# zju3dv/LoG

Measured on NVIDIA H100. Metric: gaussians_per_s_fwd_bwd, higher is better.
Workload: dtype f32

## Files before the change

### log_b200/csrc/lgr_blend.cu

```cuda
#include "lgr_common.cuh"
#include "lgr_prof.cuh"

namespace lgr {

constexpr int BLEND_THREADS = TILE_PIX;
#ifndef LGR_FWD_MIN_CTAS
#define LGR_FWD_MIN_CTAS 5
#endif
#ifndef LGR_BWD_MIN_CTAS
#define LGR_BWD_MIN_CTAS 4
#endif
#ifndef LGR_FWD6_MIN_CTAS
#define LGR_FWD6_MIN_CTAS 4
#endif
#ifndef LGR_BWD6_MIN_CTAS
#define LGR_BWD6_MIN_CTAS 3
#endif
constexpr int BATCH = 256;
constexpr unsigned FULL = 0xffffffffu;

struct SubTile {
  int x, y;
  bool inside;
};

__device__ __forceinline__ SubTile make_subtile(const View& v, int tile, int lane, int warp) {
  SubTile s;
  const int tx = tile % v.gx, ty = v.row0 + tile / v.gx;
  const int sx = tx * TILE + (warp & 1) * 8, sy = ty * TILE + (warp >> 1) * 4;
  s.x = sx + (lane & 7); s.y = sy + (lane >> 3);
  s.inside = s.x < v.W && s.y < v.H;
  return s;
}

__device__ __forceinline__ unsigned subtile_bits(const float4 r0, const float4 r1, float tx0, float ty0) {
  const float xlo = r0.x - r1.z, xhi = r0.x + r1.z, ylo = r0.y - r1.w, yhi = r0.y + r1.w;
  unsigned xm = 0u, m = 0u;
  if (xhi >= tx0 && xlo <= tx0 + 7.0f) xm |= 1u;
  if (xhi >= tx0 + 8.0f && xlo <= tx0 + 15.0f) xm |= 2u;
#pragma unroll
  for (int r = 0; r < 4; r++)
    if (yhi >= ty0 + 4.0f * r && ylo <= ty0 + 4.0f * r + 3.0f) m |= xm << (2 * r);
  return m;
}

__device__ __forceinline__ float eval_power2(const float4 r0, const float con_z, float dx, float dy) {
  const float q = __fmaf_rn(r0.z, __fmul_rn(dx, dx), __fmul_rn(con_z, __fmul_rn(dy, dy)));
  return __fmaf_rn(-0.5f, q, -__fmul_rn(r0.w, __fmul_rn(dx, dy)));
}
__device__ __forceinline__ float ex2_approx(float x) {
  float y;
  asm("ex2.approx.ftz.f32 %0, %1;" : "=f"(y) : "f"(x));
  return y;
}
__device__ __forceinline__ float eval_alpha(float opacity, float G) { return fminf(ALPHA_MAX, __fmul_rn(opacity, G)); }

__device__ __forceinline__ uint32_t smem_u32(const void* p) { return (uint32_t)__cvta_generic_to_shared(p); }
__device__ __forceinline__ float4 lds_f4(uint32_t addr) {
  float4 v;
  asm volatile("ld.shared.v4.f32 {%0, %1, %2, %3}, [%4];" : "=f"(v.x), "=f"(v.y), "=f"(v.z), "=f"(v.w) : "r"(addr));
  return v;
}
__device__ __forceinline__ float2 lds_f2(uint32_t addr) {
  float2 v;
  asm volatile("ld.shared.v2.f32 {%0, %1}, [%2];" : "=f"(v.x), "=f"(v.y) : "r"(addr));
  return v;
}
__device__ __forceinline__ uint32_t pin_reg(uint32_t v) {
  asm volatile("" : "+r"(v));
  return v;
}
__device__ __forceinline__ void red_shared_max_u32(uint32_t addr, unsigned v) {
  asm volatile("red.shared.max.u32 [%0], %1;" ::"r"(addr), "r"(v) : "memory");
}
__device__ __forceinline__ void red_shared_add_f32(uint32_t addr, float v) {
  asm volatile("red.shared.add.f32 [%0], %1;" ::"r"(addr), "f"(v) : "memory");
}
__device__ __forceinline__ void sts_f32(uint32_t addr, float v) {
  asm volatile("st.shared.f32 [%0], %1;" ::"r"(addr), "f"(v) : "memory");
}
__device__ __forceinline__ float rcp_approx(float x) {
  float y;
  asm("rcp.approx.ftz.f32 %0, %1;" : "=f"(y) : "f"(x));
  return y;
}
__device__ __forceinline__ void prefetch_l2(const float* p) {
  asm volatile("prefetch.global.L2 [%0];" ::"l"(p));
}
__device__ __forceinline__ float tf32_lo(float x) { return x - __uint_as_float(__float_as_uint(x) & 0xffffe000u); }
__device__ __forceinline__ void ldsm_x4(uint32_t addr, uint32_t& r0, uint32_t& r1, uint32_t& r2, uint32_t& r3) {
  asm volatile("ldmatrix.sync.aligned.m8n8.x4.shared.b16 {%0, %1, %2, %3}, [%4];"
               : "=r"(r0), "=r"(r1), "=r"(r2), "=r"(r3) : "r"(addr));
}
__device__ __forceinline__ void mma_tf32(float& d0, float& d1, float& d2, float& d3, uint32_t a0, uint32_t a1, uint32_t a2,
                                         uint32_t a3, uint32_t b0, uint32_t b1) {
  asm volatile("mma.sync.aligned.m16n8k8.row.col.f32.tf32.tf32.f32 {%0, %1, %2, %3}, {%4, %5, %6, %7}, {%8, %9}, {%0, %1, %2, %3};"
               : "+f"(d0), "+f"(d1), "+f"(d2), "+f"(d3) : "r"(a0), "r"(a1), "r"(a2), "r"(a3), "r"(b0), "r"(b1));
}

template <bool SIX = false>
__device__ __forceinline__ void stage_splat(float4* s_rec, unsigned char* s_bits, int slot, const float* __restrict__ splat,
                                            int id, float tx0, float ty0, const uint32_t* __restrict__ recorded = nullptr,
                                            const float* __restrict__ splat_ext = nullptr) {
  constexpr int F4 = SIX ? 4 : 3;
  const float* rec = splat + (int64_t)id * LGR_SPLAT_FLOATS;
  const float4 r0 = ldg4(rec);
  float4 r1 = ldg4(rec + 4), r2 = ldg4(rec + 8);
  float4 r3;
  if (SIX) r3 = ldg4(splat_ext + 4 * (int64_t)id);
  r2.w = __int_as_float(id);
  unsigned bits;
  if (recorded) {
    const uint32_t e = *recorded;
    bits = e & 0xffu;
    r1.z = __uint_as_float(e >> 8);
  } else {
    bits = subtile_bits(r0, r1, tx0, ty0);
  }
  s_rec[F4 * slot] = r0; s_rec[F4 * slot + 1] = r1; s_rec[F4 * slot + 2] = r2;
  if (SIX) s_rec[F4 * slot + 3] = r3;
  s_bits[slot] = (unsigned char)bits;
}

template <bool AUX, bool REC, bool SIX = false>
__global__ void __launch_bounds__(BLEND_THREADS, SIX ? LGR_FWD6_MIN_CTAS : LGR_FWD_MIN_CTAS)
blend_fwd_kernel(View v, const int32_t* __restrict__ tile_start, const int32_t* __restrict__ sorted_ids,
                 const float* __restrict__ splat, float* __restrict__ image, float* __restrict__ final_T,
                 int32_t* __restrict__ n_contrib, int32_t* __restrict__ pid_pixel, float* __restrict__ pw_pixel,
                 unsigned* __restrict__ point_weight_bits, int32_t* __restrict__ point_count) {
  constexpr int F4 = SIX ? 4 : 3;
  constexpr uint32_t RB = 16u * F4;
  __shared__ float4 s_rec[BATCH * F4];
  __shared__ unsigned s_w[AUX ? BATCH : 1];
  __shared__ unsigned char s_bits[BATCH];
  __shared__ unsigned s_cb[REC ? (BLEND_THREADS / 32) * (BATCH / 32) : 1];
  const int tile = blockIdx.x, tid = threadIdx.x, lane = tid & 31, warp = tid >> 5;
  const SubTile st = make_subtile(v, tile, lane, warp);
  const float pxf = (float)st.x, pyf = (float)st.y;
  const float tx0 = (float)((tile % v.gx) * TILE), ty0 = (float)((v.row0 + tile / v.gx) * TILE);
  const int beg = tile_start[tile], len = tile_start[tile + 1] - beg;
  const uint32_t s_w_addr = smem_u32(s_w);
  const uint32_t s_rec_addr = pin_reg(smem_u32(s_rec));

  float T = 1.0f, C0 = 0.f, C1 = 0.f, C2 = 0.f, wmax = 0.f;
  float C3 = 0.f, C4 = 0.f, C5 = 0.f;
  int last = 0, wid = -1;
  int done = st.inside ? 0 : 1;
  int id_next = tid < len ? sorted_ids[beg + tid] : -1;

  int base = 0, cnt = min(BATCH, len);
  int n_rec = 0;
  auto stage = [&]() {
    if (tid < cnt) stage_splat<SIX>(s_rec, s_bits, tid, splat, id_next, tx0, ty0, nullptr, v.splat_ext);
    else s_bits[tid] = 0;
    if (AUX) s_w[tid] = 0u;
    id_next = base + BATCH + tid < len ? sorted_ids[beg + base + BATCH + tid] : -1;
    if (id_next >= 0) prefetch_l2(splat + (int64_t)id_next * LGR_SPLAT_FLOATS);
    if (SIX && id_next >= 0) prefetch_l2(v.splat_ext + 4 * (int64_t)id_next);
  };
  if (len > 0) stage();
  while (base < len) {
    __syncthreads();
    if (REC) {
      if (lane < BATCH / 32) s_cb[warp * (BATCH / 32) + lane] = 0u;
      __syncwarp();
    }
    if (!__all_sync(FULL, done)) {
      for (int c0 = 0; c0 < cnt; c0 += 32) {
        const int e_l = c0 + lane;
        unsigned mask = __ballot_sync(FULL, (s_bits[e_l] >> warp) & 1u);
        unsigned own_w = 0u;
        unsigned took = 0u;
        while (mask) {
          const int jA = __ffs(mask) - 1;
          mask &= mask - 1;
          const bool two = mask != 0u;
          const int jB = two ? __ffs(mask) - 1 : jA;
          mask &= mask - 1;
          const uint32_t recA = s_rec_addr + RB * (uint32_t)(c0 + jA), recB = s_rec_addr + RB * (uint32_t)(c0 + jB);
          const float4 r0A = lds_f4(recA), r0B = lds_f4(recB);
          const float2 r1A = lds_f2(recA + 16u), r1B = lds_f2(recB + 16u);
          const float dxA = __fsub_rn(r0A.x, pxf), dyA = __fsub_rn(r0A.y, pyf);
          const float dxB = __fsub_rn(r0B.x, pxf), dyB = __fsub_rn(r0B.y, pyf);
          const float powerA = eval_power2(r0A, r1A.x, dxA, dyA), powerB = eval_power2(r0B, r1B.x, dxB, dyB);
          const float alphaA = eval_alpha(r1A.y, ex2_approx(powerA)), alphaB = eval_alpha(r1B.y, ex2_approx(powerB));
          float wA = 0.f, wB = 0.f;
          if (!done && powerA <= 0.0f && alphaA >= ALPHA_MIN) {
            const float test_T = __fmul_rn(T, __fsub_rn(1.0f, alphaA));
            if (test_T < T_STOP) done = 1;
            else {
              wA = alphaA * T;
              const float4 r2 = lds_f4(recA + 32u);
              C0 = fmaf(r2.x, wA, C0); C1 = fmaf(r2.y, wA, C1); C2 = fmaf(r2.z, wA, C2);
              if (SIX) {
                const float4 r3 = lds_f4(recA + 48u);
                C3 = fmaf(r3.x, wA, C3); C4 = fmaf(r3.y, wA, C4); C5 = fmaf(r3.z, wA, C5);
              }
              T = test_T;
              last = base + c0 + jA + 1;
              if (AUX && wA > wmax) { wmax = wA; wid = __float_as_int(r2.w); }
            }
          }
          if (two && !done && powerB <= 0.0f && alphaB >= ALPHA_MIN) {
            const float test_T = __fmul_rn(T, __fsub_rn(1.0f, alphaB));
            if (test_T < T_STOP) done = 1;
            else {
              wB = alphaB * T;
              const float4 r2 = lds_f4(recB + 32u);
              C0 = fmaf(r2.x, wB, C0); C1 = fmaf(r2.y, wB, C1); C2 = fmaf(r2.z, wB, C2);
              if (SIX) {
                const float4 r3 = lds_f4(recB + 48u);
                C3 = fmaf(r3.x, wB, C3); C4 = fmaf(r3.y, wB, C4); C5 = fmaf(r3.z, wB, C5);
              }
              T = test_T;
              last = base + c0 + jB + 1;
              if (AUX && wB > wmax) { wmax = wB; wid = __float_as_int(r2.w); }
            }
          }
          if (AUX) {
            const unsigned mA = __reduce_max_sync(FULL, __float_as_uint(wA));
            const unsigned mB = __reduce_max_sync(FULL, __float_as_uint(wB));
            if (lane == jA) own_w = mA;
            if (two && lane == jB) own_w = mB;
          } else if (REC) {
            if (__any_sync(FULL, wA != 0.f)) took |= 1u << jA;
            if (__any_sync(FULL, wB != 0.f)) took |= 1u << jB;
          }
        }
        if (AUX && REC) took = __ballot_sync(FULL, own_w != 0u);
        if (REC && lane == 0) s_cb[warp * (BATCH / 32) + (c0 >> 5)] = took;
        if (AUX && own_w) red_shared_max_u32(s_w_addr + 4u * e_l, own_w);
        if (__all_sync(FULL, done)) break;
      }
    }
    const int all_done = __syncthreads_and(done);
    if (AUX && tid < cnt && s_w[tid]) atomicMax(point_weight_bits + __float_as_int(s_rec[F4 * tid + 2].w), s_w[tid]);
    if (REC) {
      unsigned m = 0u;
      if (lane < BATCH / 32) {
#pragma unroll
        for (int w = 0; w < BLEND_THREADS / 32; w++) m |= s_cb[w * (BATCH / 32) + lane];
      }
      const int c = __popc(m);
      int incl = c;
#pragma unroll
      for (int d = 1; d < BATCH / 32; d <<= 1) {
        const int y = __shfl_up_sync(FULL, incl, d);
        if (lane >= d) incl += y;
      }
      const unsigned mine = __shfl_sync(FULL, m, warp);
      const int before = __shfl_sync(FULL, incl - c, warp);
      if ((mine >> lane) & 1u) {
        unsigned byte = 0u;
#pragma unroll
        for (int w = 0; w < BLEND_THREADS / 32; w++) byte |= ((s_cb[w * (BATCH / 32) + warp] >> lane) & 1u) << w;
        const int k = beg + n_rec + before + __popc(mine & ((1u << lane) - 1u));
        v.contrib_id[k] = __float_as_int(s_rec[F4 * tid + 2].w);
        v.contrib_entry[k] = byte | ((uint32_t)(base + tid) << 8);
      }
      n_rec += __shfl_sync(FULL, incl, BATCH / 32 - 1);
    }
    base += BATCH;
    if (all_done || base >= len) break;
    cnt = min(BATCH, len - base);
    stage();
  }
  if (REC && tid == 0) v.contrib_count[tile] = n_rec;
  if (st.inside) {
    const int64_t pix = (int64_t)st.y * v.W + st.x, HW = (int64_t)v.H * v.W;
    image[pix] = C0 + T * __ldg(v.bg);
    image[HW + pix] = C1 + T * __ldg(v.bg + 1);
    image[2 * HW + pix] = C2 + T * __ldg(v.bg + 2);
    if (SIX) {
      image[3 * HW + pix] = C3 + T * __ldg(v.bg + 3);
      image[4 * HW + pix] = C4 + T * __ldg(v.bg + 4);
      image[5 * HW + pix] = C5 + T * __ldg(v.bg + 5);
    }
    final_T[pix] = T;
    n_contrib[pix] = last;
    if (AUX) {
      pid_pixel[pix] = (v.pid_map && wid >= 0) ? v.pid_map[wid] : wid; pw_pixel[pix] = wmax;
      if (point_count && wid >= 0) atomicAdd(point_count + wid, 1);
    }
  }
}

constexpr int HITS = 8;
constexpr int XROW = 36;
constexpr int BWD_SMEM = BATCH * 48 + BATCH * 36 + (BLEND_THREADS / 32) * (2 * HITS * XROW + 192 + 192) * 4 + BATCH;
constexpr int BWD6_SMEM = BATCH * 64 + BATCH * 48 + (BLEND_THREADS / 32) * (2 * HITS * XROW + 384 + 192) * 4 + BATCH;

template <bool REC, bool SIX = false>
__global__ void __launch_bounds__(BLEND_THREADS, SIX ? LGR_BWD6_MIN_CTAS : LGR_BWD_MIN_CTAS)
blend_bwd_kernel(View v, const int32_t* __restrict__ tile_start, const int32_t* __restrict__ sorted_ids,
                 const float* __restrict__ splat, const float* __restrict__ image,
                 const float* __restrict__ dL_dimage, float* __restrict__ dsplat) {
  constexpr int F4 = SIX ? 4 : 3;
  constexpr uint32_t RB = 16u * F4;
  constexpr int NCH = SIX ? 6 : 3;
  constexpr int NG = 6 + NCH;
  constexpr int NCW = 64 * NCH;
  extern __shared__ float4 smem_f4[];
  float4* s_rec = smem_f4;
  float* s_g = reinterpret_cast<float*>(s_rec + BATCH * F4);
  float* s_x = s_g + BATCH * NG;
  float* s_cw = s_x + (BLEND_THREADS / 32) * 2 * HITS * XROW;
  float* s_mw = s_cw + (BLEND_THREADS / 32) * NCW;
  unsigned char* s_bits = reinterpret_cast<unsigned char*>(s_mw + (BLEND_THREADS / 32) * 192);
  const int tile = blockIdx.x, tid = threadIdx.x, lane = tid & 31, warp = tid >> 5;
  const SubTile st = make_subtile(v, tile, lane, warp);
  const float pxf = (float)st.x, pyf = (float)st.y;
  const float tx0 = (float)((tile % v.gx) * TILE), ty0 = (float)((v.row0 + tile / v.gx) * TILE);
  const int beg = tile_start[tile], len = tile_start[tile + 1] - beg;
  const uint32_t s_g_addr = pin_reg(smem_u32(s_g));
  const uint32_t s_rec_addr = pin_reg(smem_u32(s_rec));
  const uint32_t xg_addr = pin_reg(smem_u32(s_x) + (uint32_t)warp * (2 * HITS * XROW * 4));
  const uint32_t xlane_addr = pin_reg(xg_addr + 4u * (uint32_t)lane);
  const uint32_t xrow = pin_reg(xg_addr + (uint32_t)(lane & 7) * (XROW * 4) + (uint32_t)((lane >> 3) & 1) * (HITS * XROW * 4) +
                                (uint32_t)(lane >> 4) * 16u);
  const float tcx = tx0 + 7.5f, tcy = ty0 + 7.5f;
  const int g = lane >> 2, t = lane & 3;

  float Rd = 0.f, dp0 = 0.f, dp1 = 0.f, dp2 = 0.f;
  float dp3 = 0.f, dp4 = 0.f, dp5 = 0.f;
  int last = 0;
  if (st.inside) {
    const int64_t pix = (int64_t)st.y * v.W + st.x, HW = (int64_t)v.H * v.W;
    dp0 = dL_dimage[pix]; dp1 = dL_dimage[HW + pix]; dp2 = dL_dimage[2 * HW + pix];
    Rd = image[pix] * dp0 + image[HW + pix] * dp1 + image[2 * HW + pix] * dp2;
    if (SIX) {
      dp3 = dL_dimage[3 * HW + pix]; dp4 = dL_dimage[4 * HW + pix]; dp5 = dL_dimage[5 * HW + pix];
      Rd += image[3 * HW + pix] * dp3 + image[4 * HW + pix] * dp4 + image[5 * HW + pix] * dp5;
    }
    if (REC) last = v.last_contrib[pix];
  }
  const uint32_t mw_addr = pin_reg(smem_u32(s_mw) + (uint32_t)warp * (192 * 4) + (uint32_t)((min(g, 5) * 4 + t) * 8));
  for (int k = lane; k < 192; k += 32) {
    const int which = k & 1, l_ = (k >> 1) % 24, s_ = (k >> 1) / 24, t_ = l_ & 3, g_ = l_ >> 2;
    const float u = (float)((warp & 1) * 8 + t_ + 4 * which) - 7.5f, vv = (float)((warp >> 1) * 4 + s_) - 7.5f;
    const float f = g_ == 0 ? 1.f : g_ == 1 ? u : g_ == 2 ? vv : g_ == 3 ? u * u : g_ == 4 ? u * vv : vv * vv;
    s_mw[warp * 192 + k] = f;
  }
  const uint32_t cw_addr = pin_reg(smem_u32(s_cw) + (uint32_t)warp * (NCW * 4) + (uint32_t)((min(g, NCH - 1) * 4 + t) * 16));
  {
    float* cw = s_cw + warp * NCW;
    const int col = lane & 7, s = lane >> 3, tt = col & 3, which = col >> 2;
    const float dpc[6] = {dp0, dp1, dp2, dp3, dp4, dp5};
#pragma unroll
    for (int c = 0; c < NCH; c++) {
      cw[(s * 4 * NCH + c * 4 + tt) * 4 + which] = dpc[c];
      cw[(s * 4 * NCH + c * 4 + tt) * 4 + 2 + which] = tf32_lo(dpc[c]);
    }
  }
  __syncwarp();

  float T = 1.0f;
  int done = st.inside ? (REC ? (last == 0) : 0) : 1;
  const int n = REC ? v.contrib_count[tile] : len;
  const int32_t* __restrict__ ids = REC ? v.contrib_id : sorted_ids;
  int id_next = tid < len ? ids[beg + tid] : -1;
  if (tid >= n) id_next = -1;

  int base = 0, cnt = min(BATCH, n);
  auto stage = [&]() {
    if (tid < cnt) {
      stage_splat<SIX>(s_rec, s_bits, tid, splat, id_next, tx0, ty0, REC ? v.contrib_entry + beg + base + tid : nullptr,
                       v.splat_ext);
#pragma unroll
      for (int k = 0; k < NG; k++) s_g[tid * NG + k] = 0.f;
    } else {
      s_bits[tid] = 0;
    }
    id_next = base + BATCH + tid < n ? ids[beg + base + BATCH + tid] : -1;
    if (id_next >= 0) prefetch_l2(splat + (int64_t)id_next * LGR_SPLAT_FLOATS);
    if (SIX && id_next >= 0) prefetch_l2(v.splat_ext + 4 * (int64_t)id_next);
  };
  if (n > 0) stage();
  while (base < n) {
    __syncthreads();
    if (!__all_sync(FULL, done)) {
      int c0 = -32, pend = 0, my_e = 0;
      unsigned mask = 0u;
      bool fin = false;
      while (true) {
        if (mask == 0u) {
          do {
            c0 += 32;
            fin = c0 >= cnt || __all_sync(FULL, done);
            if (fin) break;
            mask = __ballot_sync(FULL, (s_bits[c0 + lane] >> warp) & 1u);
          } while (mask == 0u);
        }
        if (!fin) {
          const int jA = __ffs(mask) - 1;
          mask &= mask - 1;
          const bool two = mask != 0u;
          const int jB = two ? __ffs(mask) - 1 : jA;
          mask &= mask - 1;
          const int eA = c0 + jA, eB = c0 + jB;
          const uint32_t recA = s_rec_addr + RB * (uint32_t)eA, recB = s_rec_addr + RB * (uint32_t)eB;
          const float4 r0A = lds_f4(recA), r0B = lds_f4(recB);
          const float2 r1A = lds_f2(recA + 16u), r1B = lds_f2(recB + 16u);
          const float dxA = __fsub_rn(r0A.x, pxf), dyA = __fsub_rn(r0A.y, pyf);
          const float dxB = __fsub_rn(r0B.x, pxf), dyB = __fsub_rn(r0B.y, pyf);
          const float powerA = eval_power2(r0A, r1A.x, dxA, dyA), powerB = eval_power2(r0B, r1B.x, dxB, dyB);
          const float GA = ex2_approx(powerA), GB = ex2_approx(powerB);
          const float alphaA = eval_alpha(r1A.y, GA), alphaB = eval_alpha(r1B.y, GB);
          const float omA = __fsub_rn(1.0f, alphaA), omB = __fsub_rn(1.0f, alphaB);
          bool cA = false, cB = false;
          const float TA = T;
          float TB;
          if (REC) {
            const int iA = __float_as_int(s_rec[F4 * eA + 1].z), iB = __float_as_int(s_rec[F4 * eB + 1].z);
            cA = !done && powerA <= 0.0f && alphaA >= ALPHA_MIN;
            if (cA) T = __fmul_rn(T, omA);
            done = (iA + 1 >= last);
            TB = T;
            cB = two && !done && powerB <= 0.0f && alphaB >= ALPHA_MIN;
            if (cB) T = __fmul_rn(T, omB);
            if (two) done = (iB + 1 >= last);
          } else {
            if (!done && powerA <= 0.0f && alphaA >= ALPHA_MIN) {
              const float tt = __fmul_rn(T, omA);
              if (tt < T_STOP) done = 1; else { cA = true; T = tt; }
            }
            TB = T;
            if (two && !done && powerB <= 0.0f && alphaB >= ALPHA_MIN) {
              const float tt = __fmul_rn(T, omB);
              if (tt < T_STOP) done = 1; else { cB = true; T = tt; }
            }
          }
          const bool anyA = __any_sync(FULL, cA), anyB = __any_sync(FULL, cB);
          if (anyA) {
            float wG = 0.f, w = 0.f;
            if (cA) {
              const float4 r2 = lds_f4(recA + 32u);
              w = alphaA * TA;
              float cdot = r2.x * dp0 + r2.y * dp1 + r2.z * dp2;
              if (SIX) {
                const float4 r3 = lds_f4(recA + 48u);
                cdot += r3.x * dp3 + r3.y * dp4 + r3.z * dp5;
              }
              Rd = fmaf(-cdot, w, Rd);
              const float dL_dalpha = cdot * TA - Rd * rcp_approx(omA);
              wG = r1A.y * dL_dalpha * GA;
            }
            const uint32_t row = xlane_addr + (uint32_t)pend * (XROW * 4);
            sts_f32(row, wG); sts_f32(row + HITS * XROW * 4, w);
            if (lane == pend) my_e = eA;
            pend++;
          }
          if (anyB) {
            float wG = 0.f, w = 0.f;
            if (cB) {
              const float4 r2 = lds_f4(recB + 32u);
              w = alphaB * TB;
              float cdot = r2.x * dp0 + r2.y * dp1 + r2.z * dp2;
              if (SIX) {
                const float4 r3 = lds_f4(recB + 48u);
                cdot += r3.x * dp3 + r3.y * dp4 + r3.z * dp5;
              }
              Rd = fmaf(-cdot, w, Rd);
              const float dL_dalpha = cdot * TB - Rd * rcp_approx(omB);
              wG = r1B.y * dL_dalpha * GB;
            }
            const uint32_t row = xlane_addr + (uint32_t)pend * (XROW * 4);
            sts_f32(row, wG); sts_f32(row + HITS * XROW * 4, w);
            if (lane == pend) my_e = eB;
            pend++;
          }
        }
        if (pend >= HITS - 1 || (fin && pend > 0)) {
          __syncwarp();
          float d0 = 0.f, d1 = 0.f, z0 = 0.f, z1 = 0.f, y0 = 0.f, y1 = 0.f, d2 = 0.f, d3 = 0.f;
#pragma unroll
          for (int s = 0; s < 4; s++) {
            uint32_t a0, a1, a2, a3;
            ldsm_x4(xrow + 32u * s, a0, a1, a2, a3);
            const uint32_t l0 = __float_as_uint(tf32_lo(__uint_as_float(a0))), l1 = __float_as_uint(tf32_lo(__uint_as_float(a1)));
            const uint32_t l2 = __float_as_uint(tf32_lo(__uint_as_float(a2))), l3 = __float_as_uint(tf32_lo(__uint_as_float(a3)));
            float2 bm = make_float2(0.f, 0.f);
            float4 bc = make_float4(0.f, 0.f, 0.f, 0.f);
            if (g < 6) bm = lds_f2(mw_addr + 192u * s);
            if (g < NCH) bc = lds_f4(cw_addr + (64u * NCH) * s);
            mma_tf32(d0, d1, z0, z1, a0, a1, a2, a3, __float_as_uint(bm.x), __float_as_uint(bm.y));
            mma_tf32(y0, y1, d2, d3, a0, a1, a2, a3, __float_as_uint(bc.x), __float_as_uint(bc.y));
            mma_tf32(d0, d1, z0, z1, l0, l1, l2, l3, __float_as_uint(bm.x), __float_as_uint(bm.y));
            mma_tf32(y0, y1, d2, d3, l0, l1, l2, l3, __float_as_uint(bc.x), __float_as_uint(bc.y));
            mma_tf32(y0, y1, d2, d3, a0, a1, a2, a3, __float_as_uint(bc.z), __float_as_uint(bc.w));
          }
          const uint32_t acc = s_g_addr + (4u * NG) * (uint32_t)__shfl_sync(FULL, my_e, g);
          if (g < pend) {
            if (t < 3) { red_shared_add_f32(acc + 8u * t, d0); red_shared_add_f32(acc + 8u * t + 4u, d1); }
            if (SIX) {
              if (t < 3) { red_shared_add_f32(acc + 24u + 8u * t, d2); red_shared_add_f32(acc + 28u + 8u * t, d3); }
            } else {
              if (t < 2) red_shared_add_f32(acc + 24u + 8u * t, d2);
              if (t == 0) red_shared_add_f32(acc + 28u, d3);
            }
          }
          __syncwarp();
          pend = 0;
        }
        if (fin) break;
      }
    }
    const int all_done = __syncthreads_and(done);
    if (tid < cnt) {
      const float* m = s_g + tid * NG;
      const float M00 = m[0], M10 = m[1], M01 = m[2], M20 = m[3], M11 = m[4], M02 = m[5];
      bool nz = (M00 != 0.f) | (M10 != 0.f) | (M01 != 0.f) | (M20 != 0.f) | (M11 != 0.f) | (M02 != 0.f) |
                (m[6] != 0.f) | (m[7] != 0.f) | (m[8] != 0.f);
      if (SIX) nz |= (m[NG - 3] != 0.f) | (m[NG - 2] != 0.f) | (m[NG - 1] != 0.f);
      if (nz) {
        const float4 r0 = s_rec[F4 * tid];
        const float2 r1 = *reinterpret_cast<const float2*>(&s_rec[F4 * tid + 1]);
        const int id = __float_as_int(s_rec[F4 * tid + 2].w);
        const float X = r0.x - tcx, Y = r0.y - tcy;
        const float Sx = fmaf(X, M00, -M10), Sy = fmaf(Y, M00, -M01);
        const float Sxx = fmaf(X, fmaf(X, M00, -2.f * M10), M20);
        const float Syy = fmaf(Y, fmaf(Y, M00, -2.f * M01), M02);
        const float Sxy = fmaf(X, fmaf(Y, M00, -M01), fmaf(-Y, M10, M11));
        float4 a, b;
        a.x = -(r0.z * Sx + r0.w * Sy);
        a.y = -(r1.x * Sy + r0.w * Sx);
        a.z = -0.5f * Sxx;
        a.w = -Sxy;
        b.x = -0.5f * Syy;
        b.y = M00 / r1.y;
        b.z = m[6]; b.w = m[7];
        float4* dst = reinterpret_cast<float4*>(dsplat + (int64_t)id * LGR_GRAD_FLOATS);
        atomicAdd(dst, a);
        atomicAdd(dst + 1, b);
        if (SIX) atomicAdd(dst + 2, make_float4(m[8], m[NG - 3], m[NG - 2], m[NG - 1]));
        else atomicAdd(reinterpret_cast<float*>(dst + 2), m[8]);
      }
    }
    base += BATCH;
    if (all_done || base >= n) break;
    cnt = min(BATCH, n - base);
    stage();
  }
}

template <bool SIX>
static void launch_blend_fwd_ch(const View& v, bool rec, int ntiles, const int32_t* tile_start, const int32_t* sorted_ids,
                                const float* splat, float* image, float* final_T, int32_t* n_contrib, int32_t* pid_pixel,
                                float* pw_pixel, unsigned* pwb, int32_t* point_count, cudaStream_t st) {
  if (v.want_aux && rec)
    blend_fwd_kernel<true, true, SIX><<<ntiles, BLEND_THREADS, 0, st>>>(v, tile_start, sorted_ids, splat, image, final_T, n_contrib, pid_pixel, pw_pixel, pwb, point_count);
  else if (v.want_aux)
    blend_fwd_kernel<true, false, SIX><<<ntiles, BLEND_THREADS, 0, st>>>(v, tile_start, sorted_ids, splat, image, final_T, n_contrib, pid_pixel, pw_pixel, pwb, point_count);
  else if (rec)
    blend_fwd_kernel<false, true, SIX><<<ntiles, BLEND_THREADS, 0, st>>>(v, tile_start, sorted_ids, splat, image, final_T, n_contrib, pid_pixel, pw_pixel, pwb, point_count);
  else
    blend_fwd_kernel<false, false, SIX><<<ntiles, BLEND_THREADS, 0, st>>>(v, tile_start, sorted_ids, splat, image, final_T, n_contrib, pid_pixel, pw_pixel, pwb, point_count);
}

int launch_blend_fwd(const View& v, const int32_t* tile_start, const int32_t* sorted_ids, const float* splat,
                     float* image, float* final_T, int32_t* n_contrib, int32_t* pid_pixel, float* pw_pixel,
                     float* point_weight, int32_t* point_count, cudaStream_t st) {
  const int ntiles = v.gx * (v.row1 - v.row0);
  if (ntiles <= 0) return 0;
  ProfScope ps(K_BLEND_FWD, st);
  unsigned* pwb = reinterpret_cast<unsigned*>(point_weight);
  const bool rec = v.contrib_id != nullptr && v.contrib_entry != nullptr && v.contrib_count != nullptr;
  if (v.num_channels == 6)
    launch_blend_fwd_ch<true>(v, rec, ntiles, tile_start, sorted_ids, splat, image, final_T, n_contrib, pid_pixel, pw_pixel, pwb, point_count, st);
  else
    launch_blend_fwd_ch<false>(v, rec, ntiles, tile_start, sorted_ids, splat, image, final_T, n_contrib, pid_pixel, pw_pixel, pwb, point_count, st);
  LGR_CHECK_LAUNCH();
  return 0;
}

template <bool SIX>
static cudaError_t launch_blend_bwd_ch(const View& v, bool rec, int ntiles, const int32_t* tile_start, const int32_t* sorted_ids,
                                       const float* splat, const float* image, const float* dL_dimage, float* dsplat, cudaStream_t st) {
  constexpr int smem = SIX ? BWD6_SMEM : BWD_SMEM;
  cudaError_t e = rec ? cudaFuncSetAttribute(blend_bwd_kernel<true, SIX>, cudaFuncAttributeMaxDynamicSharedMemorySize, smem)
                      : cudaFuncSetAttribute(blend_bwd_kernel<false, SIX>, cudaFuncAttributeMaxDynamicSharedMemorySize, smem);
  if (e != cudaSuccess) return e;
  ProfScope ps(K_BLEND_BWD, st);
  if (rec) blend_bwd_kernel<true, SIX><<<ntiles, BLEND_THREADS, smem, st>>>(v, tile_start, sorted_ids, splat, image, dL_dimage, dsplat);
  else blend_bwd_kernel<false, SIX><<<ntiles, BLEND_THREADS, smem, st>>>(v, tile_start, sorted_ids, splat, image, dL_dimage, dsplat);
  return cudaSuccess;
}

int launch_blend_bwd(const View& v, const int32_t* tile_start, const int32_t* sorted_ids, const float* splat,
                     const float* image, const float* dL_dimage, float* dsplat, cudaStream_t st) {
  const int ntiles = v.gx * (v.row1 - v.row0);
  if (ntiles <= 0) return 0;
  const bool rec = v.contrib_id != nullptr && v.contrib_entry != nullptr && v.contrib_count != nullptr && v.last_contrib != nullptr;
  const cudaError_t e = v.num_channels == 6 ? launch_blend_bwd_ch<true>(v, rec, ntiles, tile_start, sorted_ids, splat, image, dL_dimage, dsplat, st)
                                            : launch_blend_bwd_ch<false>(v, rec, ntiles, tile_start, sorted_ids, splat, image, dL_dimage, dsplat, st);
  if (e != cudaSuccess) return (int)e;
  LGR_CHECK_LAUNCH();
  return 0;
}

}
```

### profiles/contrib_stats.py

```python
import argparse
import json
import os
import sys

import numpy as np
import torch

ROOT = os.path.dirname(os.path.dirname(os.path.abspath(__file__)))
sys.path.insert(0, ROOT)

BATCH = 256


def main():
    ap = argparse.ArgumentParser()
    ap.add_argument('--workload', default='10m')
    args = ap.parse_args()
    from bench import WORKLOADS, make_inputs
    from log_b200 import GaussianRasterizationSettings, rasterize_forward
    from log_b200._capi import LGR_FILTER_MAX
    n, W, H, _, deg = WORKLOADS[args.workload]
    dev = torch.device('cuda')
    cam, sc, _ = make_inputs(args.workload)
    d = {k: v.to(dev) for k, v in sc.items()}
    settings = GaussianRasterizationSettings(
        image_height=H, image_width=W, tanfovx=cam.tanfovx, tanfovy=cam.tanfovy, bg=cam.bg.to(dev), scale_modifier=1.0,
        viewmatrix=cam.viewmatrix.to(dev), projmatrix=cam.projmatrix.to(dev), sh_degree=deg, campos=cam.campos.to(dev),
        prefiltered=False, debug=False)
    *_, st = rasterize_forward(settings, d['means3D'], d['opacities'].reshape(-1), d['scales'], d['rotations'],
                               d['colors'] if deg == 0 else None, d['shs'] if deg > 0 else None, LGR_FILTER_MAX, True)
    torch.cuda.synchronize()
    count = st.contrib_lists()[2].cpu().numpy().astype(np.int64)
    start = st.tile_start.cpu().numpy().astype(np.int64)
    nc = st.n_contrib.cpu().numpy()
    gx, gy = (W + 15) // 16, (H + 15) // 16
    pad = np.zeros((gy * 16, gx * 16), np.int64)
    pad[:H, :W] = nc
    maxlast = pad.reshape(gy, 16, gx, 16).max(axis=(1, 3)).reshape(-1)
    lens = start[1:] - start[:-1]
    used = lens > 0
    b_before = np.where(used, np.maximum(1, (maxlast + BATCH - 1) // BATCH), 0)
    staged = np.minimum(lens, b_before * BATCH)
    nz_staged = count[:len(lens)]
    assert (nz_staged <= staged).all()
    b_after = (nz_staged + BATCH - 1) // BATCH
    out = {
        'workload': args.workload, 'gpu': torch.cuda.get_device_name(), 'instances': int(lens.sum()),
        'tiles': int(len(lens)), 'tiles_with_entries': int(used.sum()),
        'staged_entries': int(staged.sum()), 'nonzero_staged_entries': int(nz_staged.sum()),
        'zero_share_of_staged': float(1.0 - nz_staged.sum() / max(staged.sum(), 1)),
        'staged_share_of_list': float(staged.sum() / max(lens.sum(), 1)),
        'batches_per_tile_before': {'mean': float(b_before[used].mean()), 'max': int(b_before.max()), 'total': int(b_before.sum())},
        'batches_per_tile_after': {'mean': float(b_after[used].mean()), 'max': int(b_after.max()), 'total': int(b_after.sum())},
    }
    print(json.dumps(out))


if __name__ == '__main__':
    main()
```

Before: 1.841 billion.

## Flush per-warp gradient moments directly to global atomics instead of shared accumulation

The backward blend kernel no longer accumulates per-splat moments in a shared-memory buffer with shared atomics followed by a per-batch flush pass. Each warp now gathers its MMA results with shuffles, and one lane per hit computes the splat gradient and issues vector atomicAdds to global memory. This removes the shared gradient buffer, its zeroing and the end-of-batch flush, and reduces shared memory per block. In exchange, global atomics are issued once per warp hit instead of once per staged splat, which raises atomic traffic and contention. The profiling script gains statistics on warp hits and per-warp load imbalance.

New measurement: 1.931 billion, median of 6. +4.9%, better.

```diff
diff --git a/log_b200/csrc/lgr_blend.cu b/log_b200/csrc/lgr_blend.cu
--- a/log_b200/csrc/lgr_blend.cu
+++ b/log_b200/csrc/lgr_blend.cu
@@ -72,9 +72,6 @@
 }
 __device__ __forceinline__ void red_shared_max_u32(uint32_t addr, unsigned v) {
   asm volatile("red.shared.max.u32 [%0], %1;" ::"r"(addr), "r"(v) : "memory");
-}
-__device__ __forceinline__ void red_shared_add_f32(uint32_t addr, float v) {
-  asm volatile("red.shared.add.f32 [%0], %1;" ::"r"(addr), "f"(v) : "memory");
 }
 __device__ __forceinline__ void sts_f32(uint32_t addr, float v) {
   asm volatile("st.shared.f32 [%0], %1;" ::"r"(addr), "f"(v) : "memory");
@@ -287,8 +284,8 @@
 
 constexpr int HITS = 8;
 constexpr int XROW = 36;
-constexpr int BWD_SMEM = BATCH * 48 + BATCH * 36 + (BLEND_THREADS / 32) * (2 * HITS * XROW + 192 + 192) * 4 + BATCH;
-constexpr int BWD6_SMEM = BATCH * 64 + BATCH * 48 + (BLEND_THREADS / 32) * (2 * HITS * XROW + 384 + 192) * 4 + BATCH;
+constexpr int BWD_SMEM = BATCH * 48 + (BLEND_THREADS / 32) * (2 * HITS * XROW + 192 + 192) * 4 + BATCH;
+constexpr int BWD6_SMEM = BATCH * 64 + (BLEND_THREADS / 32) * (2 * HITS * XROW + 384 + 192) * 4 + BATCH;
 
 template <bool REC, bool SIX = false>
 __global__ void __launch_bounds__(BLEND_THREADS, SIX ? LGR_BWD6_MIN_CTAS : LGR_BWD_MIN_CTAS)
@@ -298,12 +295,10 @@
   constexpr int F4 = SIX ? 4 : 3;
   constexpr uint32_t RB = 16u * F4;
   constexpr int NCH = SIX ? 6 : 3;
-  constexpr int NG = 6 + NCH;
   constexpr int NCW = 64 * NCH;
   extern __shared__ float4 smem_f4[];
   float4* s_rec = smem_f4;
-  float* s_g = reinterpret_cast<float*>(s_rec + BATCH * F4);
-  float* s_x = s_g + BATCH * NG;
+  float* s_x = reinterpret_cast<float*>(s_rec + BATCH * F4);
   float* s_cw = s_x + (BLEND_THREADS / 32) * 2 * HITS * XROW;
   float* s_mw = s_cw + (BLEND_THREADS / 32) * NCW;
   unsigned char* s_bits = reinterpret_cast<unsigned char*>(s_mw + (BLEND_THREADS / 32) * 192);
@@ -312,13 +307,11 @@
   const float pxf = (float)st.x, pyf = (float)st.y;
   const float tx0 = (float)((tile % v.gx) * TILE), ty0 = (float)((v.row0 + tile / v.gx) * TILE);
   const int beg = tile_start[tile], len = tile_start[tile + 1] - beg;
-  const uint32_t s_g_addr = pin_reg(smem_u32(s_g));
   const uint32_t s_rec_addr = pin_reg(smem_u32(s_rec));
   const uint32_t xg_addr = pin_reg(smem_u32(s_x) + (uint32_t)warp * (2 * HITS * XROW * 4));
   const uint32_t xlane_addr = pin_reg(xg_addr + 4u * (uint32_t)lane);
   const uint32_t xrow = pin_reg(xg_addr + (uint32_t)(lane & 7) * (XROW * 4) + (uint32_t)((lane >> 3) & 1) * (HITS * XROW * 4) +
                                 (uint32_t)(lane >> 4) * 16u);
-  const float tcx = tx0 + 7.5f, tcy = ty0 + 7.5f;
   const int g = lane >> 2, t = lane & 3;
 
   float Rd = 0.f, dp0 = 0.f, dp1 = 0.f, dp2 = 0.f;
@@ -366,8 +359,6 @@
     if (tid < cnt) {
       stage_splat<SIX>(s_rec, s_bits, tid, splat, id_next, tx0, ty0, REC ? v.contrib_entry + beg + base + tid : nullptr,
                        v.splat_ext);
-#pragma unroll
-      for (int k = 0; k < NG; k++) s_g[tid * NG + k] = 0.f;
     } else {
       s_bits[tid] = 0;
     }
@@ -489,15 +480,35 @@
             mma_tf32(y0, y1, d2, d3, l0, l1, l2, l3, __float_as_uint(bc.x), __float_as_uint(bc.y));
             mma_tf32(y0, y1, d2, d3, a0, a1, a2, a3, __float_as_uint(bc.z), __float_as_uint(bc.w));
           }
-          const uint32_t acc = s_g_addr + (4u * NG) * (uint32_t)__shfl_sync(FULL, my_e, g);
-          if (g < pend) {
-            if (t < 3) { red_shared_add_f32(acc + 8u * t, d0); red_shared_add_f32(acc + 8u * t + 4u, d1); }
-            if (SIX) {
-              if (t < 3) { red_shared_add_f32(acc + 24u + 8u * t, d2); red_shared_add_f32(acc + 28u + 8u * t, d3); }
-            } else {
-              if (t < 2) red_shared_add_f32(acc + 24u + 8u * t, d2);
-              if (t == 0) red_shared_add_f32(acc + 28u, d3);
-            }
+          const float M00 = d0, M10 = d1;
+          const float M01 = __shfl_down_sync(FULL, d0, 1), M20 = __shfl_down_sync(FULL, d1, 1);
+          const float M11 = __shfl_down_sync(FULL, d0, 2), M02 = __shfl_down_sync(FULL, d1, 2);
+          const float c2 = __shfl_down_sync(FULL, d2, 1);
+          float c3 = 0.f, c4 = 0.f, c5 = 0.f;
+          if (SIX) { c3 = __shfl_down_sync(FULL, d3, 1); c4 = __shfl_down_sync(FULL, d2, 2); c5 = __shfl_down_sync(FULL, d3, 2); }
+          const int e = __shfl_sync(FULL, my_e, g);
+          if (t == 0 && g < pend) {
+            const float4 r0 = s_rec[F4 * e];
+            const float4 r1 = s_rec[F4 * e + 1];
+            const int id = __float_as_int(s_rec[F4 * e + 2].w);
+            const float X = r0.x - (tx0 + 7.5f), Y = r0.y - (ty0 + 7.5f);
+            const float Sx = fmaf(X, M00, -M10), Sy = fmaf(Y, M00, -M01);
+            const float Sxx = fmaf(X, fmaf(X, M00, -2.f * M10), M20);
+            const float Syy = fmaf(Y, fmaf(Y, M00, -2.f * M01), M02);
+            const float Sxy = fmaf(X, fmaf(Y, M00, -M01), fmaf(-Y, M10, M11));
+            float4 a, b;
+            a.x = -(r0.z * Sx + r0.w * Sy);
+            a.y = -(r1.x * Sy + r0.w * Sx);
+            a.z = -0.5f * Sxx;
+            a.w = -Sxy;
+            b.x = -0.5f * Syy;
+            b.y = M00 / r1.y;
+            b.z = d2; b.w = d3;
+            float4* dst = reinterpret_cast<float4*>(dsplat + (int64_t)id * LGR_GRAD_FLOATS);
+            atomicAdd(dst, a);
+            atomicAdd(dst + 1, b);
+            if (SIX) atomicAdd(dst + 2, make_float4(c2, c3, c4, c5));
+            else atomicAdd(reinterpret_cast<float*>(dst + 2), c2);
           }
           __syncwarp();
           pend = 0;
@@ -506,36 +517,6 @@
       }
     }
     const int all_done = __syncthreads_and(done);
-    if (tid < cnt) {
-      const float* m = s_g + tid * NG;
-      const float M00 = m[0], M10 = m[1], M01 = m[2], M20 = m[3], M11 = m[4], M02 = m[5];
-      bool nz = (M00 != 0.f) | (M10 != 0.f) | (M01 != 0.f) | (M20 != 0.f) | (M11 != 0.f) | (M02 != 0.f) |
-                (m[6] != 0.f) | (m[7] != 0.f) | (m[8] != 0.f);
-      if (SIX) nz |= (m[NG - 3] != 0.f) | (m[NG - 2] != 0.f) | (m[NG - 1] != 0.f);
-      if (nz) {
-        const float4 r0 = s_rec[F4 * tid];
-        const float2 r1 = *reinterpret_cast<const float2*>(&s_rec[F4 * tid + 1]);
-        const int id = __float_as_int(s_rec[F4 * tid + 2].w);
-        const float X = r0.x - tcx, Y = r0.y - tcy;
-        const float Sx = fmaf(X, M00, -M10), Sy = fmaf(Y, M00, -M01);
-        const float Sxx = fmaf(X, fmaf(X, M00, -2.f * M10), M20);
-        const float Syy = fmaf(Y, fmaf(Y, M00, -2.f * M01), M02);
-        const float Sxy = fmaf(X, fmaf(Y, M00, -M01), fmaf(-Y, M10, M11));
-        float4 a, b;
-        a.x = -(r0.z * Sx + r0.w * Sy);
-        a.y = -(r1.x * Sy + r0.w * Sx);
-        a.z = -0.5f * Sxx;
-        a.w = -Sxy;
-        b.x = -0.5f * Syy;
-        b.y = M00 / r1.y;
-        b.z = m[6]; b.w = m[7];
-        float4* dst = reinterpret_cast<float4*>(dsplat + (int64_t)id * LGR_GRAD_FLOATS);
-        atomicAdd(dst, a);
-        atomicAdd(dst + 1, b);
-        if (SIX) atomicAdd(dst + 2, make_float4(m[8], m[NG - 3], m[NG - 2], m[NG - 1]));
-        else atomicAdd(reinterpret_cast<float*>(dst + 2), m[8]);
-      }
-    }
     base += BATCH;
     if (all_done || base >= n) break;
     cnt = min(BATCH, n - base);
diff --git a/profiles/contrib_stats.py b/profiles/contrib_stats.py
--- a/profiles/contrib_stats.py
+++ b/profiles/contrib_stats.py
@@ -44,6 +44,18 @@
     nz_staged = count[:len(lens)]
     assert (nz_staged <= staged).all()
     b_after = (nz_staged + BATCH - 1) // BATCH
+    entry = st.contrib_lists()[1].cpu().numpy().view(np.uint32)
+    ntiles = len(lens)
+    cnt = nz_staged
+    pos = np.repeat(start[:ntiles], cnt) + (np.arange(cnt.sum()) - np.repeat(np.cumsum(cnt) - cnt, cnt))
+    byte = (entry[pos] & 0xff).astype(np.uint8)
+    bits = np.unpackbits(byte[:, None], axis=1, bitorder='little')
+    tile_of = np.repeat(np.arange(ntiles), cnt)
+    hits_tw = np.zeros((ntiles, 8), np.int64)
+    np.add.at(hits_tw, tile_of, bits.astype(np.int64))
+    busy = hits_tw.sum(axis=1) > 0
+    imb = hits_tw[busy].max(axis=1) / hits_tw[busy].mean(axis=1)
+    hits = int(hits_tw.sum())
     out = {
         'workload': args.workload, 'gpu': torch.cuda.get_device_name(), 'instances': int(lens.sum()),
         'tiles': int(len(lens)), 'tiles_with_entries': int(used.sum()),
@@ -52,6 +64,12 @@
         'staged_share_of_list': float(staged.sum() / max(lens.sum(), 1)),
         'batches_per_tile_before': {'mean': float(b_before[used].mean()), 'max': int(b_before.max()), 'total': int(b_before.sum())},
         'batches_per_tile_after': {'mean': float(b_after[used].mean()), 'max': int(b_after.max()), 'total': int(b_after.sum())},
+        'warp_hits': hits, 'warp_hits_per_entry': float(hits / max(int(cnt.sum()), 1)),
+        'vector_reds': {'per_warp_hit': 3 * hits, 'per_entry': 3 * int(cnt.sum())},
+        'slowest_warp_over_mean': {'mean': float(imb.mean()), 'p50': float(np.median(imb)), 'p90': float(np.percentile(imb, 90)),
+                                   'hit_weighted': float((hits_tw[busy].max(axis=1) * 8).sum() / max(hits, 1))},
+        'entries_per_warp_tile': {'mean': float(cnt[busy].mean()), 'max': int(cnt.max()),
+                                  'hits_per_warp_tile_mean': float(hits_tw[busy].mean())},
     }
     print(json.dumps(out))
 
```
